# utiasSTARS/pyslam

Hardware: AMD Instinct MI355X
Metric: ms/LM-iter (Jac build + J^T J + Schur solve), stereo BA @ 500k residuals (lower is better)
Workload: dtype f64

## Files before the change

include/pyslam_hip.h:

```cpp
#ifndef PYSLAM_HIP_H
#define PYSLAM_HIP_H

#include <stdint.h>

#ifdef __cplusplus
extern "C" {
#endif

typedef struct ps_problem ps_problem;

typedef struct ps_problem_desc {
    int32_t dof;
    int32_t num_poses;
    const double*  poses;
    const int32_t* pose_rid;
    int32_t num_points;
    const double*  points;
    const int32_t* point_vid;

    int64_t num_obs;
    const int32_t* obs_pose;
    const int32_t* obs_point;
    const double*  obs_uvd;
    const int32_t* obs_grp;
// ... 140 lines not shown
int ps_covariance_column(ps_problem* h, int kind, int index, int comp, double tol, int max_iters,
                         int* iters_out, double* relres_out);

#define PS_COV_DENSE_MAX_UNKNOWNS 12288
int ps_covariance_marginals(ps_problem* h, double* pose_blocks ,
                            double* point_blocks );
int ps_covariance_pose_blocks(ps_problem* h, int64_t n, const int32_t* a, const int32_t* b,
                              double* out );
int ps_covariance_cross_blocks(ps_problem* h, int64_t n, const int32_t* kind_a, const int32_t* a,
                               const int32_t* kind_b, const int32_t* b, double* out );

int ps_triangulate(ps_problem* h, int64_t n, const int32_t* vids , int refine_iters, double min_parallax_deg,
                   int write_back, double* points_out , int32_t* status_out );

int ps_get_reduced_system(ps_problem* h, int32_t* row_ptr, int32_t* col_idx,
                          double* vals, double* g);
int ps_get_landmark_factors(ps_problem* h, double* cinv , double* c );
int ps_debug_reproj_blocks(ps_problem* h, double* r , double* jpose ,
                           double* jpoint );
int ps_debug_factor_blocks(ps_problem* h, double* r, double* j1, double* j2);
int ps_debug_table_checksums(ps_problem* h, uint64_t* out, int capacity, int* count);
int ps_debug_packed_runs(ps_problem* h, int32_t* nwaves, int32_t capacity_waves, int32_t* run, int32_t* first, int32_t* lm_ptr,
                         double* sq_part);

int ps_set_option(ps_problem* h, const char* name, double value);
int ps_get_option(ps_problem* h, const char* name, double* value);

int ps_set_profiling(ps_problem* h, int enabled);
int ps_get_stage_times(ps_problem* h, double* ms , int64_t* counts, int reset);

int ps_dense_normal_solve(const double* J, const double* r, int32_t m, int32_t n,
                          double* dx, double* covariance );

int ps_sparse_normal_solve(int32_t m, int32_t n, const int32_t* j_row_ptr, const int32_t* j_col, const double* j_val,
                           const int32_t* jt_row_ptr, const int32_t* jt_col, const double* jt_val,
                           const double* r, const double* rhs, double tol, int32_t max_iters,
                           double* dx, int32_t* iters_out, double* relres_out);

int ps_sparse_normal_direct(int32_t m, int32_t n, const int32_t* j_row_ptr, const int32_t* j_col, const double* j_val,
                            const int32_t* jt_row_ptr, const int32_t* jt_col, const double* jt_val,
                            const double* r, const double* rhs, int32_t refine_steps, double* dx, double* relres_out);

int ps_debug_band_inverse(const double* a, int32_t ncb, int32_t dof, int32_t bw, int32_t chunk_nodes, float* ainv_out,
                          double* elapsed_us);
enum { PS_LDI_READ_STATE = 0, PS_LDI_READ_S32 = 1, PS_LDI_READ_X32 = 2, PS_LDI_READ_XU = 3, PS_LDI_READ_XT = 4, PS_LDI_READ_LINV = 5,
       PS_LDI_READ_COEF = 6, PS_LDI_READ_FRO = 7, PS_LDI_READ_R = 8, PS_LDI_READ_Z = 9 };
// ... 119 lines not shown
```

pyslam_amd/_native.py:

```python
import ctypes as C
import os

import numpy as np

_HERE = os.path.dirname(os.path.abspath(__file__))
LIB_PATH = os.path.join(_HERE, 'lib', 'libpyslam_hip.so')
if os.environ.get('PYSLAM_AMD_MEASURE') == '1':
    LIB_PATH = os.path.join(_HERE, 'lib', 'libpyslam_hip_measure.so')

c_i32p = C.POINTER(C.c_int32)
c_f64p = C.POINTER(C.c_double)
c_u8p = C.POINTER(C.c_uint8)
PS_NUM_STAGES = 12
STAGE_NAMES = ['landmark_pass', 'pose_pass', 'schur_pairs', 'pose_factors', 'pcg',
               'backsub', 'update', 'cost', 'iteration_total', 'cg_kernel', 'allreduce', 'pack_unpack']


class ProblemDesc(C.Structure):
    _fields_ = [
        ('dof', C.c_int32), ('num_poses', C.c_int32), ('poses', c_f64p), ('pose_rid', c_i32p),
        ('num_points', C.c_int32), ('points', c_f64p), ('point_vid', c_i32p),
        ('num_obs', C.c_int64), ('obs_pose', c_i32p), ('obs_point', c_i32p), ('obs_uvd', c_f64p),
        ('obs_grp', c_i32p),
        ('num_cams', C.c_int32), ('cams', c_f64p), ('num_stiff3', C.c_int32), ('stiff3', c_f64p),
# ... 89 lines not shown
    'ps_solve_lm': (C.c_int, [H, C.POINTER(LmOptions), C.c_double, C.c_int, c_f64p, C.c_int32, C.POINTER(C.c_int32),
                              C.POINTER(C.c_int32), C.POINTER(C.c_double), c_i32p, c_f64p, c_f64p, c_f64p]),
    'ps_gn_finish': (C.c_int, [H, C.c_int, c_f64p, c_f64p, c_f64p]),
    'ps_gn_solve_finish': (C.c_int, [H, C.c_double, C.c_int, C.c_int, c_f64p, c_f64p, c_f64p,
                                     C.POINTER(C.c_int), c_f64p]),
    'ps_set_collective': (C.c_int, [H, C.c_void_p, C.c_void_p]),
    'ps_set_segment_exchange': (C.c_int, [H, C.c_void_p, C.c_int32, C.c_int32, C.c_int64, C.c_int64, C.POINTER(C.c_int64), C.c_int64,
                                         C.POINTER(C.c_int64), C.POINTER(C.c_int64), C.POINTER(C.c_int64)]),
    'ps_shard_buffer': (C.c_int, [H, C.POINTER(C.c_void_p)]),
    'ps_gn_solve_finish_enqueue': (C.c_int, [H, C.c_double, C.c_int, C.c_int, C.c_int]),
    'ps_gn_result': (C.c_int, [H, C.POINTER(C.c_int), c_f64p, c_f64p, C.POINTER(C.c_int), c_f64p]),
    'ps_covariance_begin': (C.c_int, [H]),
    'ps_covariance_column': (C.c_int, [H, C.c_int, C.c_int, C.c_int, C.c_double, C.c_int, C.POINTER(C.c_int), c_f64p]),
    'ps_covariance_marginals': (C.c_int, [H, c_f64p, c_f64p]),
    'ps_covariance_pose_blocks': (C.c_int, [H, C.c_int64, c_i32p, c_i32p, c_f64p]),
    'ps_covariance_cross_blocks': (C.c_int, [H, C.c_int64, c_i32p, c_i32p, c_i32p, c_i32p, c_f64p]),
    'ps_triangulate': (C.c_int, [H, C.c_int64, c_i32p, C.c_int, C.c_double, C.c_int, c_f64p, c_i32p]),
    'ps_get_reduced_system': (C.c_int, [H, c_i32p, c_i32p, c_f64p, c_f64p]),
    'ps_get_landmark_factors': (C.c_int, [H, c_f64p, c_f64p]),
    'ps_debug_reproj_blocks': (C.c_int, [H, c_f64p, c_f64p, c_f64p]),
    'ps_debug_factor_blocks': (C.c_int, [H, c_f64p, c_f64p, c_f64p]),
    'ps_debug_table_checksums': (C.c_int, [H, C.POINTER(C.c_uint64), C.c_int, C.POINTER(C.c_int)]),
    'ps_debug_packed_runs': (C.c_int, [H, c_i32p, C.c_int32, c_i32p, c_i32p, c_i32p, c_f64p]),
    'ps_set_option': (C.c_int, [H, C.c_char_p, C.c_double]),
    'ps_get_option': (C.c_int, [H, C.c_char_p, c_f64p]),
    'ps_set_profiling': (C.c_int, [H, C.c_int]),
    'ps_get_stage_times': (C.c_int, [H, c_f64p, C.POINTER(C.c_int64), C.c_int]),
    'ps_ransac_transforms': (C.c_int, [c_f64p, c_f64p, C.c_int32, C.c_int32, c_f64p]),
    'ps_ransac_cost': (C.c_int, [c_f64p, C.c_int32, c_f64p, c_f64p, C.c_int32, c_f64p, C.c_double, c_u8p, c_i32p]),
    'ps_ransac_frame_to_frame': (C.c_int, [c_f64p, c_f64p, c_f64p, C.c_int32, c_i32p, C.c_int32, C.c_int32, c_f64p,
                                           C.c_double, c_f64p, c_i32p, c_i32p, c_i32p, c_f64p, c_u8p]),
    'ps_twoview_hypotheses': (C.c_int, [c_f64p, c_f64p, C.c_int32, c_i32p, C.c_int32, c_f64p, C.c_double, c_f64p, c_i32p, c_u8p]),
    'ps_twoview_score': (C.c_int, [c_f64p, C.c_int32, c_f64p, c_f64p, C.c_int32, c_f64p, C.c_double, c_u8p, c_i32p]),
    'ps_twoview_ransac': (C.c_int, [c_f64p, c_f64p, C.c_int32, c_i32p, C.c_int32, c_f64p, C.c_double, C.c_int32, c_f64p, c_f64p,
                                    c_u8p, c_i32p, c_f64p]),
    'ps_pnp_hypotheses': (C.c_int, [c_f64p, c_f64p, C.c_int32, c_i32p, C.c_int32, c_f64p, C.c_double, c_f64p, c_i32p, c_u8p]),
    'ps_pnp_score': (C.c_int, [c_f64p, C.c_int32, c_f64p, c_f64p, C.c_int32, c_f64p, C.c_double, c_u8p, c_i32p]),
    'ps_pnp_ransac': (C.c_int, [c_f64p, c_f64p, C.c_int32, c_i32p, C.c_int32, c_f64p, C.c_double, C.c_int32, c_f64p, c_u8p, c_i32p,
                                c_f64p, c_f64p]),
    'ps_sim3_hypotheses': (C.c_int, [c_f64p, c_f64p, c_f64p, c_f64p, C.c_int32, c_i32p, C.c_int32, c_f64p, C.c_double, C.c_int32,
                                     c_f64p, c_f64p, c_i32p, c_u8p]),
    'ps_sim3_score': (C.c_int, [c_f64p, C.c_int32, c_f64p, c_f64p, c_f64p, c_f64p, C.c_int32, c_f64p, C.c_double, c_u8p, c_i32p]),
    'ps_sim3_ransac': (C.c_int, [c_f64p, c_f64p, c_f64p, c_f64p, C.c_int32, c_i32p, C.c_int32, c_f64p, C.c_double, C.c_int32, C.c_int32,
                                 c_f64p, c_f64p, c_u8p, c_i32p, c_f64p]),
    'ps_photometric_create': (C.c_int, [C.POINTER(PhotoDesc), C.c_void_p, C.POINTER(H)]),
    'ps_photometric_destroy': (C.c_int, [H]),
# ... 143 lines not shown
```

pyslam_amd/csrc/ps_abi_problem.h:

```cpp


const char* ps_last_error(void) { return g_err.c_str(); }

int ps_device_count(void) {
    int n = 0;
    if (hipGetDeviceCount(&n) != hipSuccess) return 0;
    return n;
}

int ps_warm_up(void) {
    static std::once_flag once;
    static int rc = 0;
    std::call_once(once, [] {
        void* p = nullptr;
        if (hipMalloc(&p, 256) != hipSuccess) { rc = fail("hipMalloc failed (no usable HIP device?)"); return; }
        hipLaunchKernelGGL(k_zero4, dim3(1), dim3(256), 0, 0, (size_t)8, (double*)p, (size_t)0, (double*)nullptr, (size_t)0,
                           (double*)nullptr, (size_t)0, (double*)nullptr);
        double hostw[4] = {0, 0, 0, 0};
        (void)hipMemsetAsync(p, 0, 256, 0);
        (void)hipMemcpyAsync((char*)p + 128, p, 64, hipMemcpyDeviceToDevice, 0);
        (void)hipMemcpyAsync(hostw, p, sizeof(hostw), hipMemcpyDeviceToHost, 0);
        if (hipDeviceSynchronize() != hipSuccess) rc = fail("the warm-up launch failed");
        hipFree(p);
        hipFuncAttributes a;
#define PS_TOUCH(...) (void)hipFuncGetAttributes(&a, reinterpret_cast<const void*>(&__VA_ARGS__))
        PS_TOUCH(k_landmark_pass<false>); PS_TOUCH(k_landmark_pass_packed<false, false, true>); PS_TOUCH(k_landmark_pass_packed<false, true, true>); PS_TOUCH(k_backsub_packed<false, true>); PS_TOUCH(k_pose_pass<false>); PS_TOUCH(k_pose_finalize); PS_TOUCH(k_schur_pairs_db<0>);
        PS_TOUCH(k_schur_combine); PS_TOUCH(k_backsub<false>); PS_TOUCH(k_cost_reproj<false>); PS_TOUCH(k_cost_packed<false, true>); PS_TOUCH(k_reduce3); PS_TOUCH(k_reduce_partials);
        PS_TOUCH(k_copy2); PS_TOUCH(k_zero4); PS_TOUCH(k_lag_status_check);
        PS_TOUCH(k_block_jacobi_factor<6>); PS_TOUCH(k_scale_blocks<6>); PS_TOUCH(k_scale_blocks_p<6>); PS_TOUCH(k_rows_setup<6, PS_RS_REGS>); PS_TOUCH(k_rows_setup<6, PS_RS_EXACT>);
        PS_TOUCH(k_coarse_rowsums<6>); PS_TOUCH(k_coarse_matrix<6>); PS_TOUCH(k_coarse_chol<6, true>); PS_TOUCH(k_coarse_border<6>);
        PS_TOUCH(k_coarse_mreduce<6>); PS_TOUCH(k_coarse_xbuild<6>); PS_TOUCH(k_coarse_recover<6>); PS_TOUCH(k_cg_fused_lds<6, 8>);
        PS_TOUCH(k_cg_fused<6, 8>); PS_TOUCH(k_cg_unscale<6>); PS_TOUCH(k_update_poses<6>); PS_TOUCH(k_update_points);
        PS_TOUCH(k_xcoarse_rowsums<6>); PS_TOUCH(k_xcoarse_matrix<6>); PS_TOUCH(k_band_chol<6>); PS_TOUCH(k_band_inverse); PS_TOUCH(k_band_inverse_rl<false>);
        PS_TOUCH(k_band_inverse_rl<true>); PS_TOUCH(k_bp_v); PS_TOUCH(k_bp_t); PS_TOUCH(k_bp_w); PS_TOUCH(k_bp_dense_sep); PS_TOUCH(k_bp_dense);
        PS_TOUCH(k_xcg_restrict<6>); PS_TOUCH(k_xcg_f2_coarse<6, 3>); PS_TOUCH(k_xcg_fused1<6, 8, false>); PS_TOUCH(k_xcg_fused1<6, 0, true>);
        PS_TOUCH(k_xcg_fused1<6, 2, false>); PS_TOUCH(k_xcg_fused1<6, 6, false>);
        PS_TOUCH(k_factor_pass<6>); PS_TOUCH(k_factor_assemble<6>); PS_TOUCH(k_cost_factors<6>);
        PS_TOUCH(k_factor_pass<3>); PS_TOUCH(k_factor_assemble<3>); PS_TOUCH(k_cost_factors<3>); PS_TOUCH(k_block_jacobi_factor<3>);
        PS_TOUCH(k_update_poses<3>); PS_TOUCH(k_direct_solve<6>); PS_TOUCH(k_direct_solve<3>);
        PS_TOUCH(k_motion_only_solve<false>); PS_TOUCH(k_motion_only_iteration<false>);
        PS_TOUCH(k_pcg_spmv<6>); PS_TOUCH(k_pcg_spmv<3>); PS_TOUCH(k_ldi_init); PS_TOUCH(k_ldi_update); PS_TOUCH(k_ldi_gemm); PS_TOUCH(k_ldi_mirror);
        PS_TOUCH(k_ldi_ritz); PS_TOUCH(k_ldi_seed_prep); PS_TOUCH(k_ldi_fro_total); PS_TOUCH(k_ldi_pad_identity);
        PS_TOUCH(k_ldi_scaled_dense<6>); PS_TOUCH(k_ldi_sym_unscale<6>); PS_TOUCH(k_ldi_scaled_dense<3>); PS_TOUCH(k_ldi_sym_unscale<3>);
        PS_TOUCH(k_shard_pack<6>); PS_TOUCH(k_shard_unpack<6>); PS_TOUCH(k_publish); PS_TOUCH(k_cov_rhs); PS_TOUCH(k_triangulate<false>);
        PS_TOUCH(k_scale_blocks<3>); PS_TOUCH(k_rows_setup<3, PS_RS_REGS>); PS_TOUCH(k_rows_setup<3, PS_RS_EXACT>); PS_TOUCH(k_coarse_rowsums<3>); PS_TOUCH(k_coarse_matrix<3>);
        PS_TOUCH(k_coarse_chol<3, true>); PS_TOUCH(k_coarse_border<3>); PS_TOUCH(k_coarse_mreduce<3>); PS_TOUCH(k_coarse_xbuild<3>);
        PS_TOUCH(k_coarse_recover<3>); PS_TOUCH(k_cg_fused_lds<3, 8>); PS_TOUCH(k_cg_unscale<3>);
#undef PS_TOUCH
    });
// ... 206 lines not shown
    const int nv = h->nv;
    if ((long)nv + (long)h->L + 1 >= (1L << 31)) return fail("too many landmarks for 32-bit sort keys");
    if (ob.landmark_order(point_of_vid, class_of_row)) return -1;
    h->Nl = ob.Nl;
    if (h->alloc(&h->Z, (size_t)ob.Nl * PS_ZROW) || h->alloc(&h->Cinv, (size_t)nv * 6) ||
        h->alloc(&h->cvec, (size_t)nv * 3) || h->alloc(&h->dxl, (size_t)nv * 3)) return -1;
    return h->zero(h->dxl, (size_t)nv * 3 * sizeof(double));
}

static int create_pose_segments(ps_problem* h, const ps_problem_desc* d, ObsBuilder& ob) {
    const int nr = h->nr, P = h->P;
    if (h->nv >= (1 << 24) - 1) return fail("too many variable landmarks for the 24-bit slot field");
    if (ob.pose_order()) return -1;
    const std::vector<int32_t>& pcount = ob.pcount;
    const long Np = h->Np = pcount[nr];
    for (int r = 0; r < nr; ++r) h->max_pose_obs = std::max(h->max_pose_obs, pcount[r + 1] - pcount[r]);
    std::vector<PItem> pitems;
    std::vector<int32_t> pitem_ptr(nr + 1, 0);
    std::vector<int32_t> pose_of_rid(std::max(nr, 1), 0);
    for (int p = 0; p < P; ++p) if (d->pose_rid[p] >= 0) pose_of_rid[d->pose_rid[p]] = p;
    if (h->upload(&h->pose_of_rid, pose_of_rid)) return -1;
    int pchunk = Np >= 512L * 256 ? 512 : 256;
    if (const char* e = ps_env("PS_POSE_CHUNK")) pchunk = std::max(256, atoi(e) / 256 * 256);
    for (int r = 0; r < nr; ++r) {
        for (int s = pcount[r]; s < pcount[r + 1]; s += pchunk)
            pitems.push_back({r, s, std::min(s + pchunk, pcount[r + 1]), pose_of_rid[r]});
        pitem_ptr[r + 1] = (int32_t)pitems.size();
    }
    if (ob.place_sidx_p()) return -1;
    h->npitems = (int)pitems.size();
    if (h->upload(&h->pitems, pitems) || h->upload(&h->pitem_ptr, pitem_ptr) || ob.place_pobs() ||
        h->alloc(&h->ppartial, (size_t)pitems.size() * PS_NPOSE_ACC)) return -1;
    return 0;
}

static int create_pose_factors(ps_problem* h, const CreateIn& in, FactorTables& fac) {
    const ps_problem_desc* d = in.d;
    const ps_host_rows_desc* hrows = in.hrows;
    const int D = h->D, DD = D * D, PW = h->PW, P = h->P;
    const long E = fac.E = d->num_edges, Q = d->num_priors, F = fac.F = h->F = E + Q;
    std::vector<FactorGroup> fg(std::max(1, d->num_edge_groups));
    for (int gi = 0; gi < d->num_edge_groups; ++gi) {
        const double* row = d->edge_groups + 3 * gi;
        const int st = (int)row[0];
        if (st < 0 || st >= d->num_stiffd) return fail("edge group stiffness index out of range");
        std::memset(&fg[gi], 0, sizeof(FactorGroup));
// ... 246 lines not shown
```

pyslam_amd/csrc/ps_abi_solver.h:

```cpp

int ps_get_info(ps_problem* h, ps_problem_info* info) {
    if (!h || !info) return fail("null argument");
    info->dof = h->D; info->num_poses = h->P; info->num_reduced = h->nr; info->num_points = h->L;
    info->num_var_points = h->nv; info->num_obs = h->N; info->num_edges = h->F; info->num_priors = 0;
    info->reduced_nnzb = h->nnzb; info->num_pairs = h->npairs;
    info->reduce_count = ((long)h->nnzb + h->nr) / 2 * h->D * h->D + (long)h->nr * h->D + 3;
    info->device_bytes = (int64_t)h->dev_bytes;
    info->cg_restarts = h->cg_fallbacks;
    info->cg_kernel_launches = h->cg_kernel_launches;
    info->ldi_solves = h->ldi_solves; info->ldi_fallbacks = h->ldi_fallbacks; info->ldi_seeds = h->ldi_seeds;
    info->xcg_fused_solves = h->xf_solves; info->xcg_fused_fallbacks = h->xf_fallbacks;
    info->cg_persist_solves = h->cp_launches; info->cg_persist_failures = h->cp_failures;
    info->cg_persist_refused = h->cp_refused; info->persist_cus = h->persist_cus;
    info->persist_cus_needed = h->cp_ok ? h->cp_cus_needed : (h->xp_ok ? h->xp_cus_needed : 0);
    info->landmark_passes_taken_over = h->prelm_used;
    return 0;
}

int ps_eval_cost(ps_problem* h, int include_all_constant, double* cost) {
    if (!h || !cost) return fail("null argument");
    if (include_all_constant && h->fuse_cost == 1 && lm_cost_possible(h)) { if (lm_cost_pass(h, h->lin_lambda, SC_COST)) return -1; }
    else if (cost_pass(h, include_all_constant, SC_COST)) return -1;
    if (read_scalars(h)) return -1;
    *cost = h->h_scalars[SC_COST];
// ... 792 lines not shown
            hsh = 1469598103934665603ull;
            size_t i = 0;
            for (; i + 8 <= buf.size(); i += 8) { uint64_t w; std::memcpy(&w, &buf[i], 8); hsh = (hsh ^ w) * 1099511628211ull; }
            for (; i < buf.size(); ++i) hsh = (hsh ^ buf[i]) * 1099511628211ull;
        }
        out[t] = hsh;
    }
    return 0;
}

int ps_debug_packed_runs(ps_problem* h, int32_t* nwaves, int32_t capacity_waves, int32_t* run, int32_t* first, int32_t* lm_ptr, double* sq_part) {
    if (!h || !nwaves) return fail("null argument");
    if (sync(h)) return -1;
    const int nw = h->lmw_nwaves;
    *nwaves = nw;
    if ((run || first || sq_part) && capacity_waves < nw) return fail("ps_debug_packed_runs: capacity too small");
    if (sq_part && nw) HIP_OK(hipMemcpy(sq_part, h->sq_part_l, (size_t)cdiv(nw, 4) * 8, hipMemcpyDeviceToHost));
    if (run && nw) HIP_OK(hipMemcpy(run, h->lmw_run, (size_t)nw * sizeof(LmwRun), hipMemcpyDeviceToHost));
    if (first && nw) HIP_OK(hipMemcpy(first, h->lmw_first, ((size_t)nw + 1) * 4, hipMemcpyDeviceToHost));
    if (lm_ptr && h->nv > 0) HIP_OK(hipMemcpy(lm_ptr, h->lm_ptr, ((size_t)h->nv + 1) * 4, hipMemcpyDeviceToHost));
    return 0;
}

int ps_debug_ldi_read(ps_problem* h, int32_t what, double* out, int64_t capacity) {
    if (!h || !out) return fail("null argument");
    if (what == PS_LDI_READ_STATE) {
        if (capacity < 12) return fail("ps_debug_ldi_read: state record needs 12 doubles");
        const double rec[12] = {(double)h->ldi_state, (double)h->ldi_cur, (double)h->ldi_n, (double)h->ldi_np, (double)h->ldi_kp,
                                h->ldi_direct ? 1.0 : 0.0, h->ldi_fro_limit, (double)h->ldi_last_its, (double)h->ldi_seed_steps,
                                (double)h->nr, (double)h->D, h->ldi_ready ? 1.0 : 0.0};
        std::memcpy(out, rec, sizeof(rec));
        return 0;
    }
    if (!h->ldi_ready || h->ldi_seeds < 1) return fail("ps_debug_ldi_read: the lagged inverse has never been set up on this handle");
    HIP_OK(hipStreamSynchronize(h->stream));
    if (h->side) HIP_OK(hipStreamSynchronize(h->side));
    if (h->ldi_stream) HIP_OK(hipStreamSynchronize(h->ldi_stream));
    if (h->ev_ldi) HIP_OK(hipEventSynchronize(h->ev_ldi));
    const size_t n = (size_t)h->ldi_n, np = (size_t)h->ldi_np, kp = (size_t)h->ldi_kp;
    const void* src = nullptr; size_t count = 0; bool f32 = true;
    const bool seed_item = what == PS_LDI_READ_S32 || what == PS_LDI_READ_X32 || what == PS_LDI_READ_XT || what == PS_LDI_READ_LINV ||
                           what == PS_LDI_READ_COEF;
    if (seed_item && h->ldi_direct) return fail("ps_debug_ldi_read: the direct seed keeps no Newton-Schulz operands");
    const bool use_item = what == PS_LDI_READ_XU || what == PS_LDI_READ_R || what == PS_LDI_READ_Z;
    if (use_item && h->ldi_cur < 0) return fail("ps_debug_ldi_read: no inverse is in use");
    switch (what) {
// ... 32 lines not shown
        return 0;
    }
    if (!std::strcmp(name, "rows_regs")) {
        h->rows_regs = value != 0 ? 1 : 0;
        h->prelin_valid = h->prelm_valid = h->ride_valid = false;
        return 0;
    }
    if (!std::strcmp(name, "cg_persist_recover")) {
        h->cg_persist_recover = value != 0 ? 1 : 0;
        h->prelin_valid = h->prelm_valid = h->ride_valid = false;
        return 0;
    }
    if (!std::strcmp(name, "cg_persist_recover_lds")) {
        if (!(value >= 0 && value <= PS_CP_RECOVER_LDS_CAP)) return fail("cg_persist_recover_lds out of range (0 .. 146432 bytes)");
        h->cg_persist_recover_lds = (int)value;
        h->prelin_valid = h->prelm_valid = h->ride_valid = false;
        return 0;
    }
    if (!std::strcmp(name, "packed_prefetch")) {
        h->packed_prefetch = value != 0 ? 1 : 0;
        h->prelin_valid = h->prelm_valid = h->ride_valid = false;
        return 0;
    }
    h->prelin_valid = h->prelm_valid = h->ride_valid = false;
    const char* refusal = nullptr;
    const int fx = ps_option_apply(*h, name, value, &refusal);
    if (fx == PS_OPT_UNKNOWN) return fail(std::string("unknown option: ") + name);
    if (fx == PS_OPT_REFUSED) return fail(refusal);
    if (fx & PS_FX_COARSE_REBUILD) h->coarse_built = false;
    if (fx & PS_FX_DROP_FACTOR) h->lci_next = -1;
    if (fx & PS_FX_DROP_SIDE) h->side_todo = false;
    if ((fx & PS_FX_LDI_OFF) && !h->ldi_enable) { h->ldi_cur = -1; if (h->ldi_state != 1) h->ldi_state = 0; }
    if (fx & PS_FX_RELOOK_PATH) relook_path(h);
    relook_launch_gates(h);
    return 0;
}

int ps_get_option(ps_problem* h, const char* name, double* value) {
    if (!h || !name || !value) return fail("null argument");
    const std::string n(name);
    if (n == "lin_zero_list") *value = h->lin_zero_gate ? 1.0 : 0.0;
    else if (n == "lin_fills") *value = (double)h->lin_fills;
    else if (n == "lin_zero_launches") *value = (double)h->lin_zero_launches;
    else if (n == "setup_ride") *value = h->ride_gate ? 1.0 : 0.0;
    else if (n == "factor_launches") *value = (double)h->bjf_launches;
    else if (n == "factors_ridden") *value = (double)h->bjf_ridden;
    else if (n == "factor_plan_mismatches") *value = (double)h->bjf_mismatches;
    else if (n == "rows_regs") *value = (double)h->rows_regs;
    else if (n == "rows_setups") *value = (double)h->rows_setups;
    else if (n == "exact_row_setups") *value = (double)h->exact_row_setups;
    else if (n == "rows_lci_in_lds") *value = h->coarse_built && h->lagx_ok && h->rows_lci_lds ? 1.0 : 0.0;
    else if (n == "packed_prefetch") *value = (double)h->packed_prefetch;
    else if (n == "cg_persist_recover") *value = (double)h->cg_persist_recover;
    else if (n == "cg_persist_recover_lds") *value = (double)h->cg_persist_recover_lds;
    else if (n == "cg_persist_recover_need") *value = h->coarse_built && h->cp_ok ? (double)h->cp_rec_lds : 0.0;
    else if (n == "cg_persist_recovered") *value = (double)h->cp_rec_inside;
    else if (n == "cg_persist_recover_fallbacks") *value = (double)h->cp_rec_behind;
    else return fail("ps_get_option: no read-back for option: " + n);
    return 0;
}

int ps_reset_solver_state(ps_problem* h) {
    if (!h) return fail("null argument");
    h->prelin_valid = h->prelm_valid = h->ride_valid = false;
    if (!h->solver_touched) {
        static_cast<PsCostHistory&>(*h) = PsCostHistory{};
        return 0;
    }
    h->solver_touched = false;
    HIP_OK(hipStreamSynchronize(h->stream));
    if (h->side) HIP_OK(hipStreamSynchronize(h->side));
    if (h->ldi_stream) HIP_OK(hipStreamSynchronize(h->ldi_stream));
    drain_timers(h);
    static_cast<PsCarried&>(*h) = PsCarried{};
    static_cast<PsCostHistory&>(*h) = PsCostHistory{};
// ... 59 lines not shown
```

pyslam_amd/csrc/ps_core.hip:

```cpp
#include <hip/hip_runtime.h>

#include <algorithm>
#include <array>
#include <map>
#include <atomic>
#include <chrono>
#include <thread>
#include <climits>
#include <cmath>
#include <cstdio>
#include <cstring>
#include <memory>
#include <mutex>
#include <string>
#include <vector>

#include "pyslam_hip.h"
#include "ps_kernels.h"
#include "ps_ransac_core.h"
#include "ps_ransac.h"
#include "ps_k_twoview.h"
#include "ps_k_pnp.h"
#include "ps_k_sim3.h"
#include "ps_photo.h"
// ... 340 lines not shown
    typedef int (*allreduce_fn)(const void*, void*, size_t, int, int, void*, hipStream_t);
    allreduce_fn nccl_allreduce = nullptr;
    void* nccl_comm = nullptr;
    typedef int (*allgather_fn)(const void*, void*, size_t, int, void*, hipStream_t);
    allgather_fn seg_allgather = nullptr;
    int seg_world = 0;
    long seg_maxlen = 0, seg_nmine = 0, seg_ndst = 0;
    int32_t *seg_mine = nullptr, *seg_dst = nullptr, *seg_src_off = nullptr, *seg_src_ptr = nullptr;
    double *seg_in = nullptr, *seg_all = nullptr;
    double* shard_pack = nullptr;
    int32_t *up_slot = nullptr, *upT_slot = nullptr;
    long nup = 0, pack_count = 0;
    double* shard_buf = nullptr;
    bool shard_out = false;
    double *sq_part_l = nullptr, *sq_part_p = nullptr;
    bool lm_md = false;
    double *md_part_p = nullptr, *md_part_l = nullptr;
    int nmd_p = 0;
    int nsq_l = 0 , nsq_l16 = 0 , nsq_p = 0;
    int32_t* lmw_first = nullptr;
    int lmw_nwaves = 0;
    LmwRun* lmw_run = nullptr;
    int packed_prefetch = 1;
    bool ldi_ready = false;
    int ldi_n = 0, ldi_np = 0, ldi_kp = 0;
    float *ldi_S32 = nullptr, *ldi_X32 = nullptr, *ldi_R32 = nullptr, *ldi_T32 = nullptr, *ldi_Xt = nullptr, *ldi_XtT = nullptr;
    float* ldi_Xu[2] = {};
    double *ldi_x64 = nullptr, *ldi_Linv = nullptr, *ldi_r[2] = {}, *ldi_part = nullptr, *ldi_fro_part = nullptr;
    double *h_ldi_fro = nullptr, *h_ldi_fro_dev = nullptr;
    double ldi_fro_limit = 0.1;
    int2* ldi_krange = nullptr;
    bool side_poolable = false;
    hipStream_t ldi_stream = nullptr;
    double *ldi_A64 = nullptr, *ldi_Li = nullptr, *ldi_LiT = nullptr, *ldi_Tinv = nullptr; int32_t* ldi_stat = nullptr;
    float* ldi_coef = nullptr;
    long ldi_solves = 0, ldi_fallbacks = 0, ldi_seeds = 0;
    hipEvent_t ev_ldi = nullptr, ev_ldi_sread = nullptr;
    bool snap_valid = false;
    long long *h_early = nullptr, *h_early_dev = nullptr;
    long long early_seq = 0;
    bool spec_next = false, spec_enqueued = false, early_armed = false, prelin_valid = false;
    double prelin_lambda = 0.0;
    bool prelm_pending = false, prelm_valid = false;
    double prelm_lambda = 0.0;
    long long prelm_tag = 0, prelm_seq = 0, lmfail_check = 0, lin_lmfail_tag = 0;
    long long *h_lmfail = nullptr, *h_lmfail_dev = nullptr;
// ... 157 lines not shown
```

pyslam_amd/csrc/ps_host_cg.h:

```cpp

namespace {

struct StageTimer {
    ps_problem* h;
    int stage;
    hipEvent_t a = nullptr, b = nullptr;
    int slot = -1;
    StageTimer(ps_problem* h_, int st, int level = 2) : h(h_), stage(st) {
        if (h->profiling < level) return;
        if (h->profiling == 1 && h->prof_every > 1 &&
            h->prof_tick % h->prof_every != (st == PS_ST_CG_KERNEL ? h->prof_every / 2 : 0)) return;
        if (h->ev_used + 2 > h->ev_pool.size()) {
            for (int i = 0; i < 64; ++i) { hipEvent_t e; hipEventCreate(&e); h->ev_pool.push_back(e); }
        }
        slot = (int)h->ev_used;
        a = h->ev_pool[h->ev_used++];
        b = h->ev_pool[h->ev_used++];
        hipEventRecord(a, h->stream);
    }
    void stop() {
        if (!a) return;
        hipEventRecord(b, h->stream);
        h->pending.push_back({stage, slot});
        a = nullptr;
// ... 938 lines not shown
                           h->Cinv, h->cvec, h->status, h->lm_ablate, wl)
#define PS_LMP_LAUNCH(W, PF) hipLaunchKernelGGL((k_landmark_pass_packed<W, false, PF>), dim3(cdiv(h->lmw_nwaves, 4)), dim3(256), 0, h->stream, h->lmw_nwaves, \
                           h->lmw_first, h->lmw_run, h->lm_ptr, h->lm_point, h->lobs, h->poses, h->points, h->pose_rid, h->ogroups, lambda, h->Z,      \
                           h->Cinv, h->cvec, h->status, wl, (const int32_t*)nullptr, (double*)nullptr, (long long*)nullptr, 0LL)
        if (h->lm_packed && h->lmw_nwaves > 0 && !h->lm_ablate) {
            if (h->packed_prefetch) { if (h->wide_obs) PS_LMP_LAUNCH(true, true); else PS_LMP_LAUNCH(false, true); }
            else if (h->wide_obs) PS_LMP_LAUNCH(true, false); else PS_LMP_LAUNCH(false, false);
        }
        else if (h->wide_obs) PS_LM_LAUNCH(true); else PS_LM_LAUNCH(false);
#undef PS_LMP_LAUNCH
#undef PS_LM_LAUNCH
    }
    bool fin_in_combine = false, fin_in_pairs = false;
    static const bool schur_split_env = ps_env("PS_SCHUR_SPLIT") != nullptr;
    if (h->npitems > 0) {
        StageTimer t(h, PS_ST_POSE);
        const ObsWide wp{h->sidx_p, h->stiff_tab};
        const int per_xcd = h->pose_xcd ? cdiv(h->npitems, 8) : 0;
        const int nblk = per_xcd ? 8 * per_xcd : h->npitems;
        static_assert(ST_NWORDS % 2 == 0, "the status words are cleared as doubles");
        const int ntail = zero_by_list ? h->nr * 6 + 2 + (lm_here ? 0 : ST_NWORDS / 2) : 0;
        const int nzs = zero_by_list ? h->nzero_slots : 0;
        const int nzblk = zero_by_list ? cdiv((long)nzs * 36 + ntail, 256) : 0;
        if (h->wide_obs)
            hipLaunchKernelGGL(k_pose_pass<true>, dim3(nblk + nzblk), dim3(256), 0, h->stream, h->pitems, h->pobs,
                               h->poses, h->points, h->ogroups, h->Cinv, h->cvec, h->ppartial, lambda != 0.0 ? 1 : 0, wp, h->npitems, per_xcd,
                               nblk, (const int32_t*)h->zero_slots, nzs, h->S, h->g, ntail);
        else
            hipLaunchKernelGGL(k_pose_pass<false>, dim3(nblk + nzblk), dim3(256), 0, h->stream, h->pitems, h->pobs,
                               h->poses, h->points, h->ogroups, h->Cinv, h->cvec, h->ppartial, lambda != 0.0 ? 1 : 0, wp, h->npitems, per_xcd,
                               nblk, (const int32_t*)h->zero_slots, nzs, h->S, h->g, ntail);
        fin_in_combine = h->Spart && h->npair_items > 0 && !h->has_diag_tasks && h->D == 6;
        fin_in_pairs = !h->Spart && h->schur_pipeline && h->npair_items > 0 && !h->has_diag_tasks && h->D == 6 && !schur_split_env;
        if (!fin_in_combine && !fin_in_pairs)
            hipLaunchKernelGGL(k_pose_finalize, dim3(h->nr), dim3(64), 0, h->stream, h->nr, h->pitem_ptr,
                               h->ppartial, h->diag_slot, lambda, h->S, h->g);
    }
    if (h->npair_items > 0) {
        StageTimer t(h, PS_ST_SCHUR, 1);
        const bool split2 = schur_split_env;
        const int halfp = split2 ? (h->pair_per_xcd / 2 + 3) / 4 * 4 : h->pair_per_xcd;
        static const int lds_pad = ps_env("PS_SCHUR_LDS_PAD") ? atoi(ps_env("PS_SCHUR_LDS_PAD")) : 0;
        auto launch_pairs = [&](int nblk, int lds, int from, int to) {
            if (!h->schur_pipeline)
                hipLaunchKernelGGL(k_schur_pairs, dim3(nblk), dim3(256), lds, h->stream, h->pair_per_xcd, h->pair_xitems, h->pairs,
                                   h->Z, h->S, h->Spart, h->schur_ablate, from, to);
            else {
#ifdef PS_MEASURE
                auto k = h->schur_ablate == 0 ? k_schur_pairs_db<0> : h->schur_ablate == 1 ? k_schur_pairs_db<1> :
                         h->schur_ablate == 2 ? k_schur_pairs_db<2> : h->schur_ablate == 3 ? k_schur_pairs_db<3> :
                         h->schur_ablate == 4 ? k_schur_pairs_db<4> : k_schur_pairs_db<5>;
#else
                auto k = k_schur_pairs_db<0>;
#endif
// ... 224 lines not shown
```

pyslam_amd/csrc/ps_k_linearize.h:

```cpp
#pragma once

#define PS_LM_GROUP 16

PS_DEV double group16_sum(double v) {
    v = dpp_shift_add<0x111, 0xf, 0xf>(v);
    v = dpp_shift_add<0x112, 0xf, 0xf>(v);
    v = dpp_shift_add<0x114, 0xf, 0xe>(v);
    v = dpp_shift_add<0x118, 0xf, 0xc>(v);
    return __shfl(v, (int)(threadIdx.x & 63) | 15, 64);
}

#define PS_ZROW 16

PS_DEV void lm_emit_m(const ReprojEval& ev, double M00, double M10, double M11, double M20, double M21,
                      double M22, double* __restrict__ m) {
#pragma unroll
    for (int a = 0; a < 3; ++a) {
        const double w0 = ev.Jp[a] * ev.Jl[0] + ev.Jp[6 + a] * ev.Jl[3] + ev.Jp[12 + a] * ev.Jl[6];
        const double w1 = ev.Jp[a] * ev.Jl[1] + ev.Jp[6 + a] * ev.Jl[4] + ev.Jp[12 + a] * ev.Jl[7];
        const double w2 = ev.Jp[a] * ev.Jl[2] + ev.Jp[6 + a] * ev.Jl[5] + ev.Jp[12 + a] * ev.Jl[8];
        m[3 * a] = w0 * M00;
        m[3 * a + 1] = w0 * M10 + w1 * M11;
        m[3 * a + 2] = w0 * M20 + w1 * M21 + w2 * M22;
    }
// ... 254 lines not shown
            __builtin_amdgcn_wave_barrier();
            if (lane < nk) {
                double s = 0.0;
#pragma unroll 8
                for (int l = 0; l < 64; ++l) s += trw[l * 17 + lane];
                red[w][k0 + lane] = s;
            }
            __builtin_amdgcn_wave_barrier();
        }
    }
#else
#pragma unroll
    for (int k = 0; k < PS_NPOSE_ACC; ++k) {
        const double s = wave_sum(acc[k]);
        if (lane == 0) red[w][k] = s;
    }
#endif
    __syncthreads();
    if (threadIdx.x < PS_NPOSE_ACC)
        partial[(size_t)item * PS_NPOSE_ACC + threadIdx.x] =
            ((red[0][threadIdx.x] + red[1][threadIdx.x]) + red[2][threadIdx.x]) + red[3][threadIdx.x];
}

PS_DEV void pose_finalize_wave(int rid, int lane, const int32_t* __restrict__ pitem_ptr,
                               const double* __restrict__ partial, const int32_t* __restrict__ diag_slot,
                               double lambda, double* __restrict__ S, double* __restrict__ g, double* v ,
                               double* s_new = nullptr, double* g_new = nullptr)
{
    if (lane < PS_NPOSE_ACC) {
        double s = 0.0;
        for (int it = pitem_ptr[rid]; it < pitem_ptr[rid + 1]; ++it) s += partial[(size_t)it * PS_NPOSE_ACC + lane];
        v[lane] = s;
    }
    __builtin_amdgcn_wave_barrier();
    double sn = 0.0, gn = 0.0;
    if (lane < 36) {
        const int r = lane / 6, c = lane % 6;
        const int a = r < c ? r : c, b = r < c ? c : r;
        const int idx = a * 6 - (a * (a - 1)) / 2 + (b - a);
        double val = v[idx];
        if (r == c) val += lambda * v[27 + r];
        const size_t o = (size_t)diag_slot[rid] * 36 + lane;
        sn = S[o] + val;
        S[o] = sn;
    }
    if (lane < 6) { const size_t o = (size_t)rid * 6 + lane; gn = g[o] + v[21 + lane]; g[o] = gn; }
// ... 272 lines not shown
```

pyslam_amd/device.py:

```python
import ctypes as C

import numpy as np

from pyslam_amd import _native as nat


COVARIANCE_MARGINALS_LIMIT = 12288


def _solve_options(o, opt, linesearch=None):
    o.max_iters, o.allow_nondecreasing_steps = int(opt.max_iters), int(bool(opt.allow_nondecreasing_steps))
    o.max_nondecreasing_steps = int(opt.max_nondecreasing_steps)
    o.linesearch = int(bool(opt.linesearch_max_iters > 0 if linesearch is None else linesearch))
    o.min_update_norm, o.min_cost = float(opt.min_update_norm), float(opt.min_cost)
    o.min_cost_decrease, o.lm_lambda = float(opt.min_cost_decrease), float(getattr(opt, 'lm_lambda', 0.))
    return o


class DeviceProblem:
    def __init__(self, lp, stream=None, extra_pairs=None):
        lib = nat.require_gpu()
        self._lib = lib
        self.lp = lp
        self.dof = lp.dof
# ... 338 lines not shown
        rp, ci, vals, g = self.reduced_system()
        d, n = self.dof, self.nr * self.dof
        S = np.zeros((n, n))
        for r in range(self.nr):
            for k in range(rp[r], rp[r + 1]):
                S[r * d:(r + 1) * d, ci[k] * d:(ci[k] + 1) * d] = vals[k]
        return S, g

    def landmark_factors(self):
        cinv, c = np.zeros((self.nv, 6)), np.zeros((self.nv, 3))
        nat.check(self._lib.ps_get_landmark_factors(self._h, nat.f64p(cinv), nat.f64p(c)))
        return cinv, c

    def packed_runs(self):
        nw = C.c_int32(0)
        nat.check(self._lib.ps_debug_packed_runs(self._h, C.byref(nw), 0, None, None, None, None))
        n = nw.value
        run, first, lm_ptr = np.zeros((n, 4), dtype=np.int32), np.zeros(n + 1, dtype=np.int32), np.zeros(self.nv + 1, dtype=np.int32)
        sq = np.zeros((n + 3) // 4)
        i32 = lambda a: a.ctypes.data_as(C.POINTER(C.c_int32))
        nat.check(self._lib.ps_debug_packed_runs(self._h, C.byref(nw), n, i32(run), i32(first), i32(lm_ptr), nat.f64p(sq)))
        return run, first, lm_ptr, sq

    def debug_reproj_blocks(self):
        n = self.lp.num_obs
        r, jp, jl = np.zeros((n, 3)), np.zeros((n, 3, 6)), np.zeros((n, 3, 3))
        nat.check(self._lib.ps_debug_reproj_blocks(self._h, nat.f64p(r), nat.f64p(jp), nat.f64p(jl)))
        return r, jp, jl

    def debug_factor_blocks(self):
        f, d = self.lp.num_edges + self.lp.num_priors, self.lp.dof
        r, j1, j2 = np.zeros((f, d)), np.zeros((f, d, d)), np.zeros((f, d, d))
        nat.check(self._lib.ps_debug_factor_blocks(self._h, nat.f64p(r), nat.f64p(j1), nat.f64p(j2)))
        return r, j1, j2

    def debug_ldi_state(self):
        rec = np.zeros(12)
        nat.check(self._lib.ps_debug_ldi_read(self._h, 0, nat.f64p(rec), rec.size))
        keys = ('state', 'cur', 'n', 'np', 'kp', 'direct', 'fro_limit', 'last_its', 'seed_steps', 'nr', 'dof', 'ready')
        return {k: (float(v) if k == 'fro_limit' else int(v)) for k, v in zip(keys, rec)}

    def debug_ldi_read(self, what):
        s = self.debug_ldi_state()
        n, npad, kp, nr, d = s['n'], s['np'], s['kp'], s['nr'], s['dof']
        code, shape = {'S32': (1, (npad, npad)), 'X32': (2, (npad, npad)), 'Xu': (3, (npad, npad)), 'Xt': (4, (npad, kp)),
                       'Linv': (5, (nr, d, d)), 'coef': (6, (3,)), 'fro': (7, (1,)), 'r': (8, (n,)), 'z': (9, (n,))}[what]
# ... 356 lines not shown
```

Baseline: 0.2656.

## Add prefetching pose-pass kernel processing two observations per thread

Adds k_pose_pass_pf, a pose-pass variant where each thread gathers point, landmark-factor and stiffness data for up to two observations (chunk up to 512) before computing. This issues more independent loads early to hide memory latency. It also replaces the per-observation accumulation with compact 6-entry Gram terms plus a transposed LDS reduction. The diagonal/lambda path is made a template parameter, and the kernel is selected by default when the pose chunk fits. In exchange it uses more registers and LDS, and a debug accessor for pose items and partials is added.

```diff
diff --git a/include/pyslam_hip.h b/include/pyslam_hip.h
--- a/include/pyslam_hip.h
+++ b/include/pyslam_hip.h
@@ -186,6 +186,7 @@
 int ps_debug_table_checksums(ps_problem* h, uint64_t* out, int capacity, int* count);
 int ps_debug_packed_runs(ps_problem* h, int32_t* nwaves, int32_t capacity_waves, int32_t* run, int32_t* first, int32_t* lm_ptr,
                          double* sq_part);
+int ps_debug_pose_items(ps_problem* h, int32_t* nitems, int32_t capacity_items, int32_t* items, double* partial);
 
 int ps_set_option(ps_problem* h, const char* name, double value);
 int ps_get_option(ps_problem* h, const char* name, double* value);
diff --git a/pyslam_amd/_native.py b/pyslam_amd/_native.py
--- a/pyslam_amd/_native.py
+++ b/pyslam_amd/_native.py
@@ -135,6 +135,7 @@
     'ps_debug_factor_blocks': (C.c_int, [H, c_f64p, c_f64p, c_f64p]),
     'ps_debug_table_checksums': (C.c_int, [H, C.POINTER(C.c_uint64), C.c_int, C.POINTER(C.c_int)]),
     'ps_debug_packed_runs': (C.c_int, [H, c_i32p, C.c_int32, c_i32p, c_i32p, c_i32p, c_f64p]),
+    'ps_debug_pose_items': (C.c_int, [H, c_i32p, C.c_int32, c_i32p, c_f64p]),
     'ps_set_option': (C.c_int, [H, C.c_char_p, C.c_double]),
     'ps_get_option': (C.c_int, [H, C.c_char_p, c_f64p]),
     'ps_set_profiling': (C.c_int, [H, C.c_int]),
diff --git a/pyslam_amd/csrc/ps_abi_problem.h b/pyslam_amd/csrc/ps_abi_problem.h
--- a/pyslam_amd/csrc/ps_abi_problem.h
+++ b/pyslam_amd/csrc/ps_abi_problem.h
@@ -24,7 +24,7 @@
         hipFree(p);
         hipFuncAttributes a;
 #define PS_TOUCH(...) (void)hipFuncGetAttributes(&a, reinterpret_cast<const void*>(&__VA_ARGS__))
-        PS_TOUCH(k_landmark_pass<false>); PS_TOUCH(k_landmark_pass_packed<false, false, true>); PS_TOUCH(k_landmark_pass_packed<false, true, true>); PS_TOUCH(k_backsub_packed<false, true>); PS_TOUCH(k_pose_pass<false>); PS_TOUCH(k_pose_finalize); PS_TOUCH(k_schur_pairs_db<0>);
+        PS_TOUCH(k_landmark_pass<false>); PS_TOUCH(k_landmark_pass_packed<false, false, true>); PS_TOUCH(k_landmark_pass_packed<false, true, true>); PS_TOUCH(k_backsub_packed<false, true>); PS_TOUCH(k_pose_pass<false>); PS_TOUCH((k_pose_pass_pf<false, false>)); PS_TOUCH(k_pose_finalize); PS_TOUCH(k_schur_pairs_db<0>);
         PS_TOUCH(k_schur_combine); PS_TOUCH(k_backsub<false>); PS_TOUCH(k_cost_reproj<false>); PS_TOUCH(k_cost_packed<false, true>); PS_TOUCH(k_reduce3); PS_TOUCH(k_reduce_partials);
         PS_TOUCH(k_copy2); PS_TOUCH(k_zero4); PS_TOUCH(k_lag_status_check);
         PS_TOUCH(k_block_jacobi_factor<6>); PS_TOUCH(k_scale_blocks<6>); PS_TOUCH(k_scale_blocks_p<6>); PS_TOUCH(k_rows_setup<6, PS_RS_REGS>); PS_TOUCH(k_rows_setup<6, PS_RS_EXACT>);
@@ -277,6 +277,7 @@
     if (h->upload(&h->pose_of_rid, pose_of_rid)) return -1;
     int pchunk = Np >= 512L * 256 ? 512 : 256;
     if (const char* e = ps_env("PS_POSE_CHUNK")) pchunk = std::max(256, atoi(e) / 256 * 256);
+    h->pose_chunk = pchunk;
     for (int r = 0; r < nr; ++r) {
         for (int s = pcount[r]; s < pcount[r + 1]; s += pchunk)
             pitems.push_back({r, s, std::min(s + pchunk, pcount[r + 1]), pose_of_rid[r]});
diff --git a/pyslam_amd/csrc/ps_abi_solver.h b/pyslam_amd/csrc/ps_abi_solver.h
--- a/pyslam_amd/csrc/ps_abi_solver.h
+++ b/pyslam_amd/csrc/ps_abi_solver.h
@@ -838,6 +838,21 @@
     return 0;
 }
 
+int ps_debug_pose_items(ps_problem* h, int32_t* nitems, int32_t capacity_items, int32_t* items, double* partial) {
+    if (!h || !nitems) return fail("null argument");
+    if (sync(h)) return -1;
+    const int ni = h->npitems;
+    *nitems = ni;
+    if ((items || partial) && capacity_items < ni) return fail("ps_debug_pose_items: capacity too small");
+    if (items && ni) {
+        std::vector<PItem> tab(ni);
+        HIP_OK(hipMemcpy(tab.data(), h->pitems, (size_t)ni * sizeof(PItem), hipMemcpyDeviceToHost));
+        for (int k = 0; k < ni; ++k) { items[3 * k] = tab[k].rid; items[3 * k + 1] = tab[k].start; items[3 * k + 2] = tab[k].end; }
+    }
+    if (partial && ni) HIP_OK(hipMemcpy(partial, h->ppartial, (size_t)ni * PS_NPOSE_ACC * sizeof(double), hipMemcpyDeviceToHost));
+    return 0;
+}
+
 int ps_debug_ldi_read(ps_problem* h, int32_t what, double* out, int64_t capacity) {
     if (!h || !out) return fail("null argument");
     if (what == PS_LDI_READ_STATE) {
@@ -916,6 +931,11 @@
         h->prelin_valid = h->prelm_valid = h->ride_valid = false;
         return 0;
     }
+    if (!std::strcmp(name, "pose_prefetch")) {
+        h->pose_prefetch = value != 0 ? 1 : 0;
+        h->prelin_valid = h->prelm_valid = h->ride_valid = false;
+        return 0;
+    }
     h->prelin_valid = h->prelm_valid = h->ride_valid = false;
     const char* refusal = nullptr;
     const int fx = ps_option_apply(*h, name, value, &refusal);
@@ -945,6 +965,7 @@
     else if (n == "exact_row_setups") *value = (double)h->exact_row_setups;
     else if (n == "rows_lci_in_lds") *value = h->coarse_built && h->lagx_ok && h->rows_lci_lds ? 1.0 : 0.0;
     else if (n == "packed_prefetch") *value = (double)h->packed_prefetch;
+    else if (n == "pose_prefetch") *value = (double)h->pose_prefetch;
     else if (n == "cg_persist_recover") *value = (double)h->cg_persist_recover;
     else if (n == "cg_persist_recover_lds") *value = (double)h->cg_persist_recover_lds;
     else if (n == "cg_persist_recover_need") *value = h->coarse_built && h->cp_ok ? (double)h->cp_rec_lds : 0.0;
diff --git a/pyslam_amd/csrc/ps_core.hip b/pyslam_amd/csrc/ps_core.hip
--- a/pyslam_amd/csrc/ps_core.hip
+++ b/pyslam_amd/csrc/ps_core.hip
@@ -386,6 +386,8 @@
     int lmw_nwaves = 0;
     LmwRun* lmw_run = nullptr;
     int packed_prefetch = 1;
+    int pose_prefetch = 1;
+    int pose_chunk = 256;
     bool ldi_ready = false;
     int ldi_n = 0, ldi_np = 0, ldi_kp = 0;
     float *ldi_S32 = nullptr, *ldi_X32 = nullptr, *ldi_R32 = nullptr, *ldi_T32 = nullptr, *ldi_Xt = nullptr, *ldi_XtT = nullptr;
diff --git a/pyslam_amd/csrc/ps_host_cg.h b/pyslam_amd/csrc/ps_host_cg.h
--- a/pyslam_amd/csrc/ps_host_cg.h
+++ b/pyslam_amd/csrc/ps_host_cg.h
@@ -984,7 +984,14 @@
         const int ntail = zero_by_list ? h->nr * 6 + 2 + (lm_here ? 0 : ST_NWORDS / 2) : 0;
         const int nzs = zero_by_list ? h->nzero_slots : 0;
         const int nzblk = zero_by_list ? cdiv((long)nzs * 36 + ntail, 256) : 0;
-        if (h->wide_obs)
+#define PS_PPF_LAUNCH(W, D) hipLaunchKernelGGL((k_pose_pass_pf<W, D>), dim3(nblk + nzblk), dim3(256), 0, h->stream, h->pitems, h->pobs,       \
+                               h->poses, h->points, h->ogroups, h->Cinv, h->cvec, h->ppartial, wp, h->npitems, per_xcd,                  \
+                               nblk, (const int32_t*)h->zero_slots, nzs, h->S, h->g, ntail)
+        if (h->pose_prefetch && h->pose_chunk <= PS_POSE_PF_OBS) {
+            if (h->wide_obs) { if (lambda != 0.0) PS_PPF_LAUNCH(true, true); else PS_PPF_LAUNCH(true, false); }
+            else if (lambda != 0.0) PS_PPF_LAUNCH(false, true); else PS_PPF_LAUNCH(false, false);
+        }
+        else if (h->wide_obs)
             hipLaunchKernelGGL(k_pose_pass<true>, dim3(nblk + nzblk), dim3(256), 0, h->stream, h->pitems, h->pobs,
                                h->poses, h->points, h->ogroups, h->Cinv, h->cvec, h->ppartial, lambda != 0.0 ? 1 : 0, wp, h->npitems, per_xcd,
                                nblk, (const int32_t*)h->zero_slots, nzs, h->S, h->g, ntail);
@@ -992,6 +999,7 @@
             hipLaunchKernelGGL(k_pose_pass<false>, dim3(nblk + nzblk), dim3(256), 0, h->stream, h->pitems, h->pobs,
                                h->poses, h->points, h->ogroups, h->Cinv, h->cvec, h->ppartial, lambda != 0.0 ? 1 : 0, wp, h->npitems, per_xcd,
                                nblk, (const int32_t*)h->zero_slots, nzs, h->S, h->g, ntail);
+#undef PS_PPF_LAUNCH
         fin_in_combine = h->Spart && h->npair_items > 0 && !h->has_diag_tasks && h->D == 6;
         fin_in_pairs = !h->Spart && h->schur_pipeline && h->npair_items > 0 && !h->has_diag_tasks && h->D == 6 && !schur_split_env;
         if (!fin_in_combine && !fin_in_pairs)
diff --git a/pyslam_amd/csrc/ps_k_linearize.h b/pyslam_amd/csrc/ps_k_linearize.h
--- a/pyslam_amd/csrc/ps_k_linearize.h
+++ b/pyslam_amd/csrc/ps_k_linearize.h
@@ -300,6 +300,147 @@
             ((red[0][threadIdx.x] + red[1][threadIdx.x]) + red[2][threadIdx.x]) + red[3][threadIdx.x];
 }
 
+template <bool WIDE, bool DIAG>
+PS_DEV void pose_obs_compact(const Se3& T, const LObs& o, const double* __restrict__ pw, const double* __restrict__ m,
+                             double c0, double c1, double c2, int v, const ObsGroup* __restrict__ groups, int gfirst_id,
+                             const ObsGroup& gfirst, const double* __restrict__ Sl,
+                             double* __restrict__ G, double* __restrict__ t3, double* __restrict__ pc, double* __restrict__ dg) {
+    ReprojEval ev;
+    reproj_eval_obs_fetched<true, true, WIDE>(T, pw, &o.u, groups, PS_GRP_OF(o), gfirst_id, gfirst, Sl, ev);
+    {
+        const double* J = ev.Jp;
+        G[0] = J[0] * J[0] + J[6] * J[6] + J[12] * J[12];
+        G[1] = J[0] * J[1] + J[6] * J[7] + J[12] * J[13];
+        G[2] = J[0] * J[2] + J[6] * J[8] + J[12] * J[14];
+        G[3] = J[1] * J[1] + J[7] * J[7] + J[13] * J[13];
+        G[4] = J[1] * J[2] + J[7] * J[8] + J[13] * J[14];
+        G[5] = J[2] * J[2] + J[8] * J[8] + J[14] * J[14];
+#pragma unroll
+        for (int a = 0; a < 3; ++a) t3[a] = J[a] * ev.r[0] + J[6 + a] * ev.r[1] + J[12 + a] * ev.r[2];
+    }
+    if (DIAG) {
+        double d21[21];
+#pragma unroll
+        for (int k = 0; k < 21; ++k) d21[k] = 0.0;
+        pose_sandwich(G, ev.pc, d21);
+        dg[0] = d21[0]; dg[1] = d21[6]; dg[2] = d21[11]; dg[3] = d21[15]; dg[4] = d21[18]; dg[5] = d21[20];
+    }
+    if (v >= 0) {
+        double m9[9];
+        lm_emit_m(ev, m[0], m[1], m[2], m[3], m[4], m[5], m9);
+        G[0] -= m9[0] * m9[0] + m9[1] * m9[1] + m9[2] * m9[2];
+        G[1] -= m9[0] * m9[3] + m9[1] * m9[4] + m9[2] * m9[5];
+        G[2] -= m9[0] * m9[6] + m9[1] * m9[7] + m9[2] * m9[8];
+        G[3] -= m9[3] * m9[3] + m9[4] * m9[4] + m9[5] * m9[5];
+        G[4] -= m9[3] * m9[6] + m9[4] * m9[7] + m9[5] * m9[8];
+        G[5] -= m9[6] * m9[6] + m9[7] * m9[7] + m9[8] * m9[8];
+#pragma unroll
+        for (int a = 0; a < 3; ++a) t3[a] += m9[3 * a] * c0 + m9[3 * a + 1] * c1 + m9[3 * a + 2] * c2;
+    }
+    pc[0] = ev.pc[0]; pc[1] = ev.pc[1]; pc[2] = ev.pc[2];
+}
+
+PS_DEV double pose_cross_sub(double acc, double a, double b, double c, double d) {
+#pragma clang fp contract(off)
+    return acc - __builtin_fma(a, b, -(c * d));
+}
+
+template <bool DIAG>
+PS_DEV void pose_acc_add(const double* __restrict__ G, const double* __restrict__ t3, const double* __restrict__ pc,
+                         const double* __restrict__ dg, double* __restrict__ acc) {
+    if (DIAG) { acc[27] += dg[0]; acc[28] += dg[1]; acc[29] += dg[2]; acc[30] += dg[3]; acc[31] += dg[4]; acc[32] += dg[5]; }
+    pose_sandwich(G, pc, acc);
+    acc[21] -= t3[0]; acc[22] -= t3[1]; acc[23] -= t3[2];
+    acc[24] = pose_cross_sub(acc[24], pc[1], t3[2], pc[2], t3[1]);
+    acc[25] = pose_cross_sub(acc[25], pc[2], t3[0], pc[0], t3[2]);
+    acc[26] = pose_cross_sub(acc[26], pc[0], t3[1], pc[1], t3[0]);
+}
+
+template <bool WIDE>
+PS_DEV void pose_obs_gather(const LObs& o, int si, const double* __restrict__ points, const double* __restrict__ Cinv,
+                            const double* __restrict__ cvec, const ObsWide& wide, double* __restrict__ pw, double* __restrict__ m,
+                            double* __restrict__ c, double* __restrict__ Sl) {
+    const int v = PS_POSE_OF(o) - 1;
+    pw[0] = points[3 * (size_t)o.point]; pw[1] = points[3 * (size_t)o.point + 1]; pw[2] = points[3 * (size_t)o.point + 2];
+    if (v >= 0) {
+        const double* ci = Cinv + 6 * (size_t)v;
+#pragma unroll
+        for (int k = 0; k < 6; ++k) m[k] = ci[k];
+        c[0] = cvec[3 * (size_t)v]; c[1] = cvec[3 * (size_t)v + 1]; c[2] = cvec[3 * (size_t)v + 2];
+    }
+    if (WIDE) {
+        const double* sp = wide.stiff + 9 * (size_t)si;
+#pragma unroll
+        for (int k = 0; k < 9; ++k) Sl[k] = sp[k];
+    }
+}
+
+#define PS_POSE_PF_OBS 512
+template <bool WIDE, bool DIAG>
+__global__ __launch_bounds__(256) __attribute__((amdgpu_waves_per_eu((WIDE || DIAG) ? 3 : 4, 8))) void k_pose_pass_pf(
+    const PItem* __restrict__ items, const LObs* __restrict__ pobs, const double* __restrict__ poses,
+    const double* __restrict__ points, const ObsGroup* __restrict__ groups, const double* __restrict__ Cinv,
+    const double* __restrict__ cvec, double* __restrict__ partial, ObsWide wide, int nitems, int per_xcd,
+    int zero_first, const int32_t* __restrict__ zero_slots, int nzero_slots, double* __restrict__ S, double* __restrict__ ztail, int ntail)
+{
+    __shared__ double red[4][PS_NPOSE_ACC];
+    __shared__ double tr[4][64 * 17];
+    if ((int)blockIdx.x >= zero_first) {
+        const int e = ((int)blockIdx.x - zero_first) * 256 + (int)threadIdx.x, ns = 36 * nzero_slots;
+        if (e < ns) { const int k = e / 36; S[(size_t)zero_slots[k] * 36 + (e - 36 * k)] = 0.0; }
+        else if (e - ns < ntail) ztail[e - ns] = 0.0;
+        return;
+    }
+    const int item = per_xcd > 0 ? (int)(blockIdx.x & 7) * per_xcd + (int)(blockIdx.x >> 3) : (int)blockIdx.x;
+    if (item >= nitems) return;
+    const PItem it = items[item];
+    const int w = threadIdx.x >> 6, lane = threadIdx.x & 63;
+    const int ia = it.start + (int)threadIdx.x, ib = ia + 256;
+    const bool ha = ia < it.end, hb = ib < it.end;
+    const Se3 T = se3_load(poses + 12 * (size_t)it.pad);
+    LObs oa = {0.0, 0.0, 0.0, 0, 0}, ob = {0.0, 0.0, 0.0, 0, 0};
+    int sa = 0, sb = 0;
+    if (ha) { oa = pobs[ia]; if (WIDE) sa = wide.sidx[ia]; }
+    if (hb) { ob = pobs[ib]; if (WIDE) sb = wide.sidx[ib]; }
+    double pwa[3], ma[6] = {0, 0, 0, 0, 0, 0}, ca[3] = {0.0, 0.0, 0.0}, Sla[9];
+    double pwb[3], mb[6] = {0, 0, 0, 0, 0, 0}, cb[3] = {0.0, 0.0, 0.0}, Slb[9];
+    double Ga[6], ta[3], pca[3], da[6], Gb[6], tb[3], pcb[3], db[6];
+    if (ha) {
+        pose_obs_gather<WIDE>(oa, sa, points, Cinv, cvec, wide, pwa, ma, ca, Sla);
+        if (hb) pose_obs_gather<WIDE>(ob, sb, points, Cinv, cvec, wide, pwb, mb, cb, Slb);
+        const int g0 = __builtin_amdgcn_readfirstlane((int)PS_GRP_OF(oa));
+        const ObsGroup g = obs_group_fetch(groups, g0);
+        pose_obs_compact<WIDE, DIAG>(T, oa, pwa, ma, ca[0], ca[1], ca[2], PS_POSE_OF(oa) - 1, groups, g0, g, Sla, Ga, ta, pca, da);
+        if (hb) pose_obs_compact<WIDE, DIAG>(T, ob, pwb, mb, cb[0], cb[1], cb[2], PS_POSE_OF(ob) - 1, groups, g0, g, Slb, Gb, tb, pcb, db);
+    }
+    double acc[PS_NPOSE_ACC];
+#pragma unroll
+    for (int k = 0; k < PS_NPOSE_ACC; ++k) acc[k] = 0.0;
+    if (ha) pose_acc_add<DIAG>(Ga, ta, pca, da, acc);
+    if (hb) pose_acc_add<DIAG>(Gb, tb, pcb, db, acc);
+    {
+        double* trw = tr[w];
+#pragma unroll
+        for (int h2 = 0; h2 < 2; ++h2) {
+            const int k0 = 17 * h2, nk = h2 ? PS_NPOSE_ACC - 17 : 17;
+#pragma unroll
+            for (int k = 0; k < 17; ++k) if (k < nk) trw[lane * 17 + k] = acc[k0 + k];
+            __builtin_amdgcn_wave_barrier();
+            if (lane < nk) {
+                double s = 0.0;
+#pragma unroll 8
+                for (int l = 0; l < 64; ++l) s += trw[l * 17 + lane];
+                red[w][k0 + lane] = s;
+            }
+            __builtin_amdgcn_wave_barrier();
+        }
+    }
+    __syncthreads();
+    if (threadIdx.x < PS_NPOSE_ACC)
+        partial[(size_t)item * PS_NPOSE_ACC + threadIdx.x] =
+            ((red[0][threadIdx.x] + red[1][threadIdx.x]) + red[2][threadIdx.x]) + red[3][threadIdx.x];
+}
+
 PS_DEV void pose_finalize_wave(int rid, int lane, const int32_t* __restrict__ pitem_ptr,
                                const double* __restrict__ partial, const int32_t* __restrict__ diag_slot,
                                double lambda, double* __restrict__ S, double* __restrict__ g, double* v ,
diff --git a/pyslam_amd/device.py b/pyslam_amd/device.py
--- a/pyslam_amd/device.py
+++ b/pyslam_amd/device.py
@@ -384,6 +384,14 @@
         nat.check(self._lib.ps_debug_packed_runs(self._h, C.byref(nw), n, i32(run), i32(first), i32(lm_ptr), nat.f64p(sq)))
         return run, first, lm_ptr, sq
 
+    def pose_items(self):
+        ni = C.c_int32(0)
+        nat.check(self._lib.ps_debug_pose_items(self._h, C.byref(ni), 0, None, None))
+        n = ni.value
+        items, partial = np.zeros((n, 3), dtype=np.int32), np.zeros((n, 33))
+        nat.check(self._lib.ps_debug_pose_items(self._h, C.byref(ni), n, items.ctypes.data_as(C.POINTER(C.c_int32)), nat.f64p(partial)))
+        return items, partial
+
     def debug_reproj_blocks(self):
         n = self.lp.num_obs
         r, jp, jl = np.zeros((n, 3)), np.zeros((n, 3, 6)), np.zeros((n, 3, 3))
```

Result: faster. 0.2620, median of 6 (-1.4%).
